# Sachin-A/TraceWeaver

Measured on NVIDIA H100. Metric: spans/sec reconstructed (in+out spans of all solved services), higher is better.
Workload: dtype int64 timestamps, f64 log-likelihoods

## Files before the change

traceweaver_b200/csrc/tw_gmm.cu:

```cuda
#include "tw_kernels.cuh"

namespace tw {

constexpr double kRegCovar = 1e-6;
constexpr double kEmTol = 1e-3;
constexpr int kEmMaxIter = 100;
constexpr int kKmMaxIter = 300;
constexpr double kKmTol = 1e-4;
constexpr double kDblEps = 2.220446049250313e-16;
constexpr int KC = TW_GMM_MAX_COMP;
constexpr unsigned kFull = 0xffffffffu;

#ifdef TW_PROFILE_PHASES
__device__ unsigned long long g_gmm_phase[16];
#define TW_GPHASE_BEGIN long long _gp_t0 = clock64()
#define TW_GPHASE_RESET _gp_t0 = clock64()
#define TW_GPHASE(k)                                                               \
  do {                                                                             \
    if ((threadIdx.x & 31) == 0) {                                                 \
      long long _now = clock64();                                                  \
      atomicAdd(&g_gmm_phase[k], (unsigned long long)(_now - _gp_t0));             \
      _gp_t0 = _now;                                                               \
    }                                                                              \
  } while (0)
#define TW_GCOUNT(k, v)                                                            \
  do {                                                                             \
    if ((threadIdx.x & 31) == 0) atomicAdd(&g_gmm_phase[k], (unsigned long long)(v)); \
  } while (0)
#else
#define TW_GPHASE_BEGIN do { } while (0)
#define TW_GPHASE_RESET do { } while (0)
#define TW_GPHASE(k) do { } while (0)
#define TW_GCOUNT(k, v) do { } while (0)
#endif

__device__ unsigned long long g_gmm_em_evals;

__device__ __forceinline__ double wsum(double v) {
#pragma unroll
  for (int d = 16; d > 0; d >>= 1) v += __shfl_xor_sync(kFull, v, d);
  return v;
}

__device__ __forceinline__ int trials_for_k(int k) { return k < 3 ? 2 : 3; }
__device__ __forceinline__ int draws_for_k(int k) { return 1 + (k - 1) * trials_for_k(k); }

__device__ __forceinline__ double sq_dist(double c, double c2, double x, double x2) {
  double d = dadd(dadd(dmul(-2.0, dmul(c, x)), c2), x2);
  return d > 0.0 ? d : 0.0;
}

struct Fit {
  double mu[KC], pc[KC], logpc[KC], logw[KC];
};

struct Near { double d; int j; };
__device__ __forceinline__ Near near_min(Near a, Near b) { return b.d < a.d ? b : a; }
template <int K>
__device__ __forceinline__ int nearest(const double* cen, double x) {
  Near v[KC];
#pragma unroll
  for (int j = 0; j < KC; ++j) {
    v[j].j = j;
    v[j].d = j < K ? dadd(dmul(cen[j], cen[j]), dmul(-2.0, dmul(x, cen[j]))) : 0.0;
  }
  if (K == 1) return 0;
  if (K == 2) return near_min(v[0], v[1]).j;
  if (K == 3) return near_min(near_min(v[0], v[1]), v[2]).j;
  if (K == 4) return near_min(near_min(v[0], v[1]), near_min(v[2], v[3])).j;
  return near_min(near_min(near_min(v[0], v[1]), near_min(v[2], v[3])), v[4]).j;
}

template <class F>
__device__ __forceinline__ void sweep2(const double* __restrict__ x, int n, F&& f) {
  int i = threadIdx.x & 31;
  double a = i < n ? x[i] : 0.0;
  double b = i + 32 < n ? x[i + 32] : 0.0;
  for (int s = 0; i < n; i += 64, s += 2) {
    const double x0 = a, x1 = b;
    const bool v1 = i + 32 < n;
    a = i + 64 < n ? x[i + 64] : 0.0;
    b = i + 96 < n ? x[i + 96] : 0.0;
    f(x0, x1, v1, s);
  }
}

template <int K>
__device__ __forceinline__ void seed_centres(const double* __restrict__ x, int n, double mean,
                                             const double* __restrict__ draws, double* cen) {
  const int lane = threadIdx.x & 31;
  const int k = K;
  TW_GPHASE_BEGIN;
#pragma unroll
  for (int j = 0; j < KC; ++j) cen[j] = 0.0;
  {
    double u = draws[0];
    double un = u * (double)n;
    int id = (int)un;
    if (fabs(un - rint(un)) < 1e-6) {
      double p = 1.0 / (double)n, last = 0.0, c = 0.0;
      for (int i = 0; i < n; ++i) last += p;
      id = n - 1;
      for (int i = 0; i < n; ++i) { c += p; if (c / last > u) { id = i; break; } }
    }
    if (id > n - 1) id = n - 1;
    cen[0] = x[id] - mean;
  }
  const int trials = trials_for_k(k);
  double pot = 0.0;
  {
    double part = 0.0, c2 = cen[0] * cen[0];
    for (int i = lane; i < n; i += 32) { double xi = x[i] - mean; part += sq_dist(cen[0], c2, xi, xi * xi); }
    pot = wsum(part);
  }
  for (int ci = 1; ci < k; ++ci) {
    double rv[3];
    int cand[3];
    for (int t = 0; t < 3; ++t) { rv[t] = t < trials ? draws[1 + (ci - 1) * trials + t] * pot : 0.0; cand[t] = n - 1; }
    bool found[3] = {false, false, false};
    double carry = 0.0;
    for (int base = 0; base < n; base += 32) {
      int i = base + lane;
      double cl = 0.0;
      if (i < n) {
        double xi = x[i] - mean, x2 = xi * xi;
        cl = sq_dist(cen[0], cen[0] * cen[0], xi, x2);
        for (int j = 1; j < ci; ++j) { double d = sq_dist(cen[j], cen[j] * cen[j], xi, x2); cl = d < cl ? d : cl; }
      }
      double incl = cl;
#pragma unroll
      for (int d = 1; d < 32; d <<= 1) {
        double o = __shfl_up_sync(kFull, incl, d);
        if (lane >= d) incl += o;
      }
      incl += carry;
      for (int t = 0; t < trials; ++t) {
        if (found[t]) continue;
        unsigned m = __ballot_sync(kFull, i < n && incl >= rv[t]);
        if (m) { cand[t] = base + __ffs(m) - 1; found[t] = true; }
      }
      carry = __shfl_sync(kFull, incl, 31);
      if (found[0] && (trials < 2 || found[1]) && (trials < 3 || found[2])) break;
    }
    double cc[3], part[3] = {0.0, 0.0, 0.0};
    for (int t = 0; t < 3; ++t) cc[t] = x[cand[t]] - mean;
    for (int i = lane; i < n; i += 32) {
      double xi = x[i] - mean, x2 = xi * xi;
      double cl = sq_dist(cen[0], cen[0] * cen[0], xi, x2);
      for (int j = 1; j < ci; ++j) { double d = sq_dist(cen[j], cen[j] * cen[j], xi, x2); cl = d < cl ? d : cl; }
      for (int t = 0; t < trials; ++t) {
        double d = sq_dist(cc[t], cc[t] * cc[t], xi, x2);
        part[t] += d < cl ? d : cl;
      }
    }
    int best = 0;
    double bp = wsum(part[0]);
    for (int t = 1; t < trials; ++t) {
      double pt = wsum(part[t]);
      if (pt < bp) { bp = pt; best = t; }
    }
    cen[ci] = cc[best];
    pot = bp;
  }
  TW_GPHASE(0);
}

template <int K>
__device__ __forceinline__ void lloyd_centres(const double* __restrict__ x, int n, double mean, double tol,
                                              const double* cen_in, double* cen_out) {
  const int lane = threadIdx.x & 31;
  const int k = K;
  TW_GPHASE_BEGIN;
  double cen[KC];
#pragma unroll
  for (int j = 0; j < KC; ++j) cen[j] = cen_in[j];
  double prev[KC];
#pragma unroll
  for (int j = 0; j < KC; ++j) prev[j] = cen[j];
  bool have_prev = false, strict = false;
  const bool packed = n <= 1024;
  unsigned long long lab_lo = 0ull, lab_hi = 0ull;
  for (int it = 0; it < kKmMaxIter; ++it) {
    double sx[KC];
    int cnt_i[KC];
#pragma unroll
    for (int j = 0; j < KC; ++j) { sx[j] = 0.0; cnt_i[j] = 0; }
    bool changed = !have_prev;
    if (packed) {
      sweep2(x, n, [&](double x0, double x1, bool v1, int s) {
#pragma unroll
        for (int h = 0; h < 2; ++h) {
          const double xi = (h ? x1 : x0) - mean;
          const bool valid = h ? v1 : true;
          const int lab = nearest<K>(cen, xi);
          const int sl = s + h;
          const unsigned sh = (unsigned)(sl & 15) * 4u;
          const bool hi = sl >= 16;
          const unsigned long long w = hi ? lab_hi : lab_lo;
          changed |= valid && (int)((w >> sh) & 15ull) != lab;
          const unsigned long long nw = valid ? (w & ~(15ull << sh)) | ((unsigned long long)lab << sh) : w;
          lab_lo = hi ? lab_lo : nw;
          lab_hi = hi ? nw : lab_hi;
#pragma unroll
          for (int j = 0; j < K; ++j) {
            const bool m = valid && j == lab;
            sx[j] += m ? xi : 0.0;
            cnt_i[j] += m ? 1 : 0;
          }
        }
      });
    } else {
      for (int i = lane; i < n; i += 32) {
        const double xi = x[i] - mean;
        const int lab = nearest<K>(cen, xi);
        if (have_prev && nearest<K>(prev, xi) != lab) changed = true;
#pragma unroll
        for (int j = 0; j < K; ++j) {
          const bool m = j == lab;
          sx[j] += m ? xi : 0.0;
          cnt_i[j] += m ? 1 : 0;
        }
      }
    }
    if (!have_prev) changed = true;
    double cnt[KC];
#pragma unroll
    for (int j = 0; j < KC; ++j) cnt[j] = (double)__reduce_add_sync(kFull, cnt_i[j]);
    changed = __any_sync(kFull, changed);
#pragma unroll
    for (int j = 0; j < KC; ++j) sx[j] = wsum(sx[j]);
    for (int j = 0; j < k; ++j) {
      if (cnt[j] != 0.0) continue;
      double fd = -1.0;
      int fi = 0x7fffffff;
      for (int i = lane; i < n; i += 32) {
        double xi = x[i] - mean;
        const int nl = nearest<K>(cen, xi);
        double cn = cen[0];
#pragma unroll
        for (int q = 1; q < KC; ++q) cn = q == nl ? cen[q] : cn;
        double d = xi - cn;
        d *= d;
        if (d > fd) { fd = d; fi = i; }
      }
#pragma unroll
      for (int d = 16; d > 0; d >>= 1) {
        double od = __shfl_xor_sync(kFull, fd, d);
        int oi = __shfl_xor_sync(kFull, fi, d);
        if (od > fd || (od == fd && oi < fi)) { fd = od; fi = oi; }
      }
      double xf = x[fi] - mean;
      int ol = nearest<K>(cen, xf);
#pragma unroll
      for (int q = 0; q < KC; ++q) {
        if (q == ol) { sx[q] -= xf; cnt[q] -= 1.0; }
        if (q == j) { sx[q] = xf; cnt[q] = 1.0; }
      }
    }
    double shift_tot = 0.0;
#pragma unroll
    for (int j = 0; j < KC; ++j) {
      prev[j] = cen[j];
      if (j < k) {
        double nc = cnt[j] > 0.0 ? sx[j] * (1.0 / cnt[j]) : sx[j];
        double d = fabs(nc - cen[j]);
        shift_tot += d * d;
        cen[j] = nc;
      }
    }
    have_prev = true;
    TW_GCOUNT(5, 1);
    if (!changed) { strict = true; break; }
    if (shift_tot <= tol) break;
  }
#pragma unroll
  for (int j = 0; j < KC; ++j) cen_out[j] = strict ? prev[j] : cen[j];
  TW_GPHASE(1);
}

template <bool FULL>
__device__ __forceinline__ bool params_from_stats(Fit& f, int k, int n, const double* nk, const double* mup,
                                                  const double* S2, double shift, bool init) {
  double tot = 0.0;
  bool ok = true;
#pragma unroll
  for (int c = 0; c < KC; ++c)
    if (c < k) tot += nk[c];
#pragma unroll
  for (int c = 0; c < KC; ++c) {
    if (c < k) {
      double cov = FULL ? S2[c] / nk[c] + kRegCovar : S2[c] / nk[c] - mup[c] * mup[c] + kRegCovar;
      if (!(cov > 0.0)) ok = false;
      f.mu[c] = mup[c] + shift;
      f.pc[c] = 1.0 / sqrt(cov);
      f.logpc[c] = log(f.pc[c]);
      f.logw[c] = log(init ? nk[c] / (double)n : nk[c] / tot);
    }
  }
  return ok;
}

template <int K, bool FULL>
__device__ __forceinline__ double estep(const Fit& f, const double* __restrict__ tab, double x, double* a,
                                        double* amax_out) {
  double amax = -INFINITY;
#pragma unroll
  for (int c = 0; c < K; ++c) {
#ifdef TW_GMM_FUSED
    const double y = (x - f.mu[c]) * f.pc[c];
    a[c] = fma(-0.5 * y, y, (f.logpc[c] - 0.5 * TW_LOG_2PI) + f.logw[c]);
#else
    double lp;
    if (FULL) {
      double y = dsub(dmul(x, f.pc[c]), dmul(f.mu[c], f.pc[c]));
      lp = dmul(y, y);
    } else {
      double prec = dmul(f.pc[c], f.pc[c]);
      lp = dadd(dsub(dmul(dmul(f.mu[c], f.mu[c]), prec), dmul(2.0, dmul(x, dmul(f.mu[c], prec)))),
                dmul(dmul(x, x), prec));
    }
    a[c] = dadd(dadd(dmul(-0.5, dadd(TW_LOG_2PI, lp)), f.logpc[c]), f.logw[c]);
#endif
    amax = a[c] > amax ? a[c] : amax;
  }
  double t = 0.0;
#pragma unroll
  for (int c = 0; c < K; ++c) {
    const double d = a[c] - amax;
    const double e = exp_neg(tab, d);
    a[c] = d >= -40.0 ? e : 0.0;
    t += a[c];
  }
  *amax_out = amax;
  return t;
}

struct LogSum {
  double acc = 0.0, prod = 1.0;
  int cnt = 0;
  __device__ __forceinline__ void add(double t, double amax) {
    acc += amax;
    prod *= t;
    if (++cnt == 128) { acc += log(prod); prod = 1.0; cnt = 0; }
  }
  __device__ __forceinline__ double total() const { return acc + log(prod); }
};

template <int K, bool FULL>
__device__ __forceinline__ bool em_fit(const double* __restrict__ x, int n, double mean, const double* cen,
                                       const double* __restrict__ tab, Fit& f, bool want_score, double* score) {
  const int lane = threadIdx.x & 31;
  const int k = K;
  if (n < 2 || n < k) return false;
  const double shift = FULL ? mean : 0.0;
  double S0[KC], S1[KC], S2[KC], nk[KC], mup[KC];
  TW_GPHASE_BEGIN;
  {
    TW_GCOUNT(7, 1);
#pragma unroll
    for (int c = 0; c < KC; ++c) { S0[c] = 0.0; S1[c] = 0.0; S2[c] = 0.0; }
    sweep2(x, n, [&](double x0, double x1, bool v1, int) {
#pragma unroll
      for (int h = 0; h < 2; ++h) {
        const double xi = h ? x1 : x0;
        const int lab = (h ? v1 : true) ? nearest<K>(cen, xi - mean) : -1;
        const double xs = xi - shift, xs2 = xs * xs;
#pragma unroll
        for (int c = 0; c < K; ++c) {
          const bool m = c == lab;
          S0[c] += m ? 1.0 : 0.0;
          S1[c] += m ? xs : 0.0;
          S2[c] += m ? xs2 : 0.0;
        }
      }
    });
#pragma unroll
    for (int c = 0; c < KC; ++c) {
      nk[c] = wsum(S0[c]) + 10.0 * kDblEps;
      mup[c] = wsum(S1[c]) / nk[c];
      S2[c] = wsum(S2[c]);
    }
    if (FULL) {
#pragma unroll
      for (int c = 0; c < KC; ++c) S2[c] = 0.0;
      sweep2(x, n, [&](double x0, double x1, bool v1, int) {
#pragma unroll
        for (int h = 0; h < 2; ++h) {
          const double xi = h ? x1 : x0;
          const int lab = (h ? v1 : true) ? nearest<K>(cen, xi - mean) : -1;
          const double xs = xi - shift;
#pragma unroll
          for (int c = 0; c < K; ++c) {
            const double d = xs - mup[c];
            S2[c] += c == lab ? d * d : 0.0;
          }
        }
      });
#pragma unroll
      for (int c = 0; c < KC; ++c) S2[c] = wsum(S2[c]);
    }
  }
  if (!params_from_stats<FULL>(f, k, n, nk, mup, S2, shift, true)) return false;
  TW_GPHASE(2);
  double lower = -INFINITY;
  int em_sweeps = 0;
  for (int it = 1; it <= kEmMaxIter; ++it) {
    const double prev = lower;
    LogSum ls;
#pragma unroll
    for (int c = 0; c < KC; ++c) { S0[c] = 0.0; S1[c] = 0.0; S2[c] = 0.0; }
    for (int i = lane; i < n; i += 32) {
      double xi = x[i], a[KC], amax;
      const double t = estep<K, FULL>(f, tab, xi, a, &amax);
      ls.add(t, amax);
      const double inv = 1.0 / t;
#pragma unroll
      for (int c = 0; c < K; ++c) {
        const double r = a[c] * inv;
        S0[c] += r;
        if (FULL) {
          const double dx = xi - f.mu[c];
          const double rd = r * dx;
          S1[c] += rd;
          S2[c] += rd * dx;
        } else {
          S1[c] += r * xi;
          S2[c] += r * (xi * xi);
        }
      }
    }
    lower = wsum(ls.total()) / (double)n;
#pragma unroll
    for (int c = 0; c < KC; ++c) {
      if (c < K) {
        nk[c] = wsum(S0[c]) + 10.0 * kDblEps;
        const double s1 = wsum(S1[c]);
        S2[c] = wsum(S2[c]);
        if (FULL) {
          const double delta = s1 / nk[c];
          S2[c] -= delta * s1;
          if (S2[c] < 0.0) S2[c] = 0.0;
          mup[c] = (f.mu[c] + delta) - shift;
        } else {
          mup[c] = s1 / nk[c];
        }
      }
    }
    if (!params_from_stats<FULL>(f, k, n, nk, mup, S2, shift, false)) {
      if (lane == 0) atomicAdd(&g_gmm_em_evals, (unsigned long long)it * (unsigned long long)n * K);
      return false;
    }
    TW_GCOUNT(6, 1);
    em_sweeps = it;
    if (fabs(lower - prev) < kEmTol) break;
  }
  if (lane == 0) atomicAdd(&g_gmm_em_evals, (unsigned long long)(em_sweeps + (want_score ? 1 : 0)) * (unsigned long long)n * K);
  TW_GPHASE(3);
  if (want_score) {
    LogSum ls;
    for (int i = lane; i < n; i += 32) {
      double a[KC], amax;
      const double t = estep<K, FULL>(f, tab, x[i], a, &amax);
      ls.add(t, amax);
    }
    *score = wsum(ls.total()) / (double)n;
  }
  TW_GPHASE(4);
  return true;
}

__global__ void __launch_bounds__(128)
k_gmm_prep(int n_terms, const int64_t* __restrict__ term_sample_off, const double* __restrict__ delays,
           const int32_t* __restrict__ counts, int32_t* __restrict__ max_n, double* __restrict__ mean_var) {
  const int t = (int)((blockIdx.x * (unsigned)blockDim.x + threadIdx.x) >> 5);
  const int lane = threadIdx.x & 31;
  if (t >= n_terms) return;
  const double* x = delays + term_sample_off[t];
  const int n = counts[t];
  double set[KC];
  int ns = 0;
  double part = 0.0;
  for (int i = lane; i < n; i += 32) {
    double v = x[i];
    part += v;
    bool seen = false;
#pragma unroll
    for (int q = 0; q < KC; ++q)
      if (q < ns && set[q] == v) seen = true;
    if (!seen && ns < KC) {
#pragma unroll
      for (int q = 0; q < KC; ++q)
        if (q == ns) set[q] = v;
      ++ns;
    }
  }
  double mset[KC];
  int mn = 0;
  for (int src = 0; src < 32 && mn < KC; ++src) {
    int sn = __shfl_sync(kFull, ns, src);
    for (int q = 0; q < KC; ++q) {
      double v = __shfl_sync(kFull, set[q < KC ? q : 0], src);
      if (q >= sn || mn >= KC) continue;
      bool seen = false;
#pragma unroll
      for (int r = 0; r < KC; ++r)
        if (r < mn && mset[r] == v) seen = true;
      if (!seen) {
#pragma unroll
        for (int r = 0; r < KC; ++r)
          if (r == mn) mset[r] = v;
        ++mn;
      }
    }
  }
  double mean = n > 0 ? wsum(part) / (double)n : 0.0;
  double p2 = 0.0;
  for (int i = lane; i < n; i += 32) { double d = x[i] - mean; p2 += d * d; }
  double var = n > 0 ? wsum(p2) / (double)n : 0.0;
  if (lane == 0) {
    max_n[t] = n > 0 ? mn : 0;
    mean_var[2 * t] = mean;
    mean_var[2 * t + 1] = var;
  }
}

__global__ void k_gmm_skip(int n_problems, const int32_t* __restrict__ prob_ep_off,
                           const int32_t* __restrict__ ep_term_off, const int32_t* __restrict__ term_order,
                           const int32_t* __restrict__ max_n, const uint32_t* __restrict__ prob_base_skip,
                           uint32_t* __restrict__ rng_skip) {
  int p = blockIdx.x * blockDim.x + threadIdx.x;
  if (p >= n_problems) return;
  int t0 = ep_term_off[prob_ep_off[p]], t1 = ep_term_off[prob_ep_off[p + 1]];
  uint32_t pos = prob_base_skip ? prob_base_skip[p] : 0u;
  for (int q = t0; q < t1; ++q) {
    int t = term_order ? term_order[q] : q;
    rng_skip[t] = pos;
    int mn = max_n[t];
    for (int k = 1; k <= mn; ++k) pos += (uint32_t)draws_for_k(k);
  }
}

__global__ void k_gmm_draws(int n_problems, const int32_t* __restrict__ prob_ep_off,
                            const int32_t* __restrict__ ep_term_off, const int32_t* __restrict__ max_n,
                            uint32_t* __restrict__ prob_draws) {
  int p = blockIdx.x * blockDim.x + threadIdx.x;
  if (p >= n_problems) return;
  uint32_t pos = 0;
  for (int t = ep_term_off[prob_ep_off[p]]; t < ep_term_off[prob_ep_off[p + 1]]; ++t)
    for (int k = 1; k <= max_n[t]; ++k) pos += (uint32_t)draws_for_k(k);
  prob_draws[p] = pos;
}

#ifndef TW_GMM_MINB
#define TW_GMM_MINB 1
#endif

struct FitSel {
  const int32_t* list;
  const uint32_t* hist;
  const int32_t* max_n;
  const uint32_t* rng_skip;
  const double* stream;
  int stream_len;
  int n_terms;
};

template <int K>
__device__ __forceinline__ bool select_fit(const FitSel& sel, const int32_t* __restrict__ counts, int* t_out,
                                           const double** draws_out, int* err_flag) {
  const unsigned w = (blockIdx.x * (unsigned)blockDim.x + threadIdx.x) >> 5;
  int t;
  const double* draws;
  if (sel.list) {
    if (w >= sel.hist[K]) return false;
    uint32_t off = 0;
#pragma unroll
    for (int q = 1; q < K; ++q) off += sel.hist[q];
    t = sel.list[off + w];
    draws = sel.stream;
  } else {
    if (w >= (unsigned)sel.n_terms) return false;
    t = (int)w;
    if (K > sel.max_n[t]) return false;
    uint32_t pos = sel.rng_skip[t];
#pragma unroll
    for (int q = 1; q < K; ++q) pos += (uint32_t)draws_for_k(q);
    if ((int)pos + draws_for_k(K) > sel.stream_len) {
      if (err_flag && (threadIdx.x & 31) == 0) atomicMin(err_flag, (int)TW_ERR_RANGE_LIMIT);
      return false;
    }
    draws = sel.stream + pos;
  }
  const int n = counts[t];
  if (n < 2 || n < K) return false;
  *t_out = t;
  *draws_out = draws;
  return true;
}

template <int K>
__global__ void __launch_bounds__(128)
k_gmm_seed(FitSel sel, const int64_t* __restrict__ term_sample_off, const double* __restrict__ delays,
           const int32_t* __restrict__ counts, const double* __restrict__ mean_var, double* __restrict__ cen_out,
           int* __restrict__ err_flag) {
  int t;
  const double* draws;
  if (!select_fit<K>(sel, counts, &t, &draws, err_flag)) return;
  double cen[KC];
  seed_centres<K>(delays + term_sample_off[t], counts[t], mean_var[2 * t], draws, cen);
  if ((threadIdx.x & 31) == 0) {
#pragma unroll
    for (int j = 0; j < K; ++j) cen_out[(size_t)t * KC + j] = cen[j];
  }
}

template <int K>
__global__ void __launch_bounds__(128)
k_gmm_lloyd(FitSel sel, const int64_t* __restrict__ term_sample_off, const double* __restrict__ delays,
            const int32_t* __restrict__ counts, const double* __restrict__ mean_var, double* __restrict__ cen_io) {
  int t;
  const double* draws;
  if (!select_fit<K>(sel, counts, &t, &draws, nullptr)) return;
  double cen[KC], out[KC];
#pragma unroll
  for (int j = 0; j < KC; ++j) cen[j] = j < K ? cen_io[(size_t)t * KC + j] : 0.0;
  lloyd_centres<K>(delays + term_sample_off[t], counts[t], mean_var[2 * t], mean_var[2 * t + 1] * kKmTol, cen, out);
  if ((threadIdx.x & 31) == 0) {
#pragma unroll
    for (int j = 0; j < K; ++j) cen_io[(size_t)t * KC + j] = out[j];
  }
}

template <int K>
__global__ void __launch_bounds__(128, TW_GMM_MINB)
k_gmm_bic(FitSel sel, const int64_t* __restrict__ term_sample_off, const double* __restrict__ delays,
          const int32_t* __restrict__ counts, const double* __restrict__ mean_var,
          const double* __restrict__ cen_in, double* __restrict__ bic_out) {
  __shared__ double tab[64];
  load_exp_table(tab);
  const int w = (int)((blockIdx.x * (unsigned)blockDim.x + threadIdx.x) >> 5);
  if (w >= sel.n_terms) return;
  double bic = INFINITY;
  int t;
  const double* draws;
  if (select_fit<K>(sel, counts, &t, &draws, nullptr)) {
    const int n = counts[t];
    double cen[KC];
#pragma unroll
    for (int j = 0; j < KC; ++j) cen[j] = j < K ? cen_in[(size_t)t * KC + j] : 0.0;
    Fit f;
    double sc = 0.0;
    if (em_fit<K, false>(delays + term_sample_off[t], n, mean_var[2 * t], cen, tab, f, true, &sc))
      bic = -2.0 * sc * (double)n + (double)(3 * K - 1) * log((double)n);
  }
  if ((threadIdx.x & 31) == 0) bic_out[(size_t)w * KC + (K - 1)] = bic;
}

__global__ void k_gmm_select(int n_terms, const int32_t* __restrict__ max_n, const double* __restrict__ bic,
                             int32_t* __restrict__ best_k_out, uint32_t* __restrict__ hist,
                             double* __restrict__ mix_out, int32_t* __restrict__ n_selected_out) {
  const int t = blockIdx.x * blockDim.x + threadIdx.x;
  if (t >= n_terms) return;
  int best_k = 0;
  double best = INFINITY;
  for (int k = 1; k <= max_n[t]; ++k) {
    double b = bic[(size_t)t * KC + (k - 1)];
    if (b < best) { best = b; best_k = k; }
  }
  best_k_out[t] = best_k;
  if (best_k > 0) atomicAdd(&hist[best_k], 1u);
  else {
    double* rec = mix_out + (size_t)t * TW_MIX_REC;
    for (int q = 0; q < TW_MIX_REC; ++q) rec[q] = 0.0;
    rec[2] = 0.001;
    rec[3] = log(0.001);
    if (n_selected_out) n_selected_out[t] = 0;
  }
}

__global__ void k_gmm_group(int n_terms, const int32_t* __restrict__ best_k, const uint32_t* __restrict__ hist,
                            uint32_t* __restrict__ cursor, int32_t* __restrict__ list) {
  const int t = blockIdx.x * blockDim.x + threadIdx.x;
  if (t >= n_terms) return;
  const int k = best_k[t];
  if (k <= 0) return;
  uint32_t off = 0;
  for (int q = 1; q < k; ++q) off += hist[q];
  list[off + atomicAdd(&cursor[k], 1u)] = t;
}

template <int K>
__global__ void __launch_bounds__(128, TW_GMM_MINB)
k_gmm_final(FitSel sel, const int64_t* __restrict__ term_sample_off, const double* __restrict__ delays,
            const int32_t* __restrict__ counts, const double* __restrict__ mean_var,
            const double* __restrict__ cen_in, double* __restrict__ mix_out, int32_t* __restrict__ n_selected_out) {
  __shared__ double tab[64];
  load_exp_table(tab);
  const unsigned w = (blockIdx.x * (unsigned)blockDim.x + threadIdx.x) >> 5;
  if (w >= sel.hist[K]) return;
  uint32_t off = 0;
#pragma unroll
  for (int q = 1; q < K; ++q) off += sel.hist[q];
  const int t = sel.list[off + w];
  const int lane = threadIdx.x & 31;
  const int n = counts[t];
  double cen[KC];
#pragma unroll
  for (int j = 0; j < KC; ++j) cen[j] = j < K ? cen_in[(size_t)t * KC + j] : 0.0;
  Fit f;
  const bool ok = em_fit<K, true>(delays + term_sample_off[t], n, mean_var[2 * t], cen, tab, f, false, nullptr);
  if (lane == 0) {
    double* rec = mix_out + (size_t)t * TW_MIX_REC;
    for (int q = 0; q < TW_MIX_REC; ++q) rec[q] = 0.0;
    if (ok) {
      rec[0] = (double)K;
#pragma unroll
      for (int c = 0; c < K; ++c) {
        rec[1 + c] = f.pc[c];
        rec[6 + c] = f.mu[c] * f.pc[c];
        rec[11 + c] = f.logpc[c];
        rec[16 + c] = f.logw[c];
      }
    } else {
      rec[2] = 0.001;
      rec[3] = log(0.001);
    }
    if (n_selected_out) n_selected_out[t] = ok ? K : 0;
  }
}

__global__ void __launch_bounds__(256)
k_fp64_peak(int iters, double* __restrict__ sink) {
  double a0 = threadIdx.x * 1e-9, a1 = a0 + 1e-3, a2 = a0 + 2e-3, a3 = a0 + 3e-3, a4 = a0 + 4e-3, a5 = a0 + 5e-3,
         a6 = a0 + 6e-3, a7 = a0 + 7e-3;
  const double m = 0.9999999, c = 1e-7;
  for (int i = 0; i < iters; ++i) {
    a0 = fma(a0, m, c); a1 = fma(a1, m, c); a2 = fma(a2, m, c); a3 = fma(a3, m, c);
    a4 = fma(a4, m, c); a5 = fma(a5, m, c); a6 = fma(a6, m, c); a7 = fma(a7, m, c);
  }
  const double r = ((a0 + a1) + (a2 + a3)) + ((a4 + a5) + (a6 + a7));
  if (r == 123.456) sink[0] = r;
}

cudaError_t launch_fp64_peak(int blocks, int iters, double* sink, cudaStream_t s, int64_t& launches) {
  k_fp64_peak<<<blocks, 256, 0, s>>>(iters, sink);
  return after_launch(launches);
}

cudaError_t gmm_work_read(unsigned long long* out, bool reset) {
  cudaError_t e = cudaMemcpyFromSymbol(out, g_gmm_em_evals, sizeof(unsigned long long));
  if (e != cudaSuccess) return e;
  if (reset) {
    const unsigned long long z = 0;
    e = cudaMemcpyToSymbol(g_gmm_em_evals, &z, sizeof z);
  }
  return e;
}

#ifdef TW_PROFILE_PHASES
extern "C" int tw_debug_gmm_phases(unsigned long long* out16, int reset) {
  cudaError_t e = cudaMemcpyFromSymbol(out16, g_gmm_phase, sizeof(unsigned long long) * 16);
  if (e != cudaSuccess) return -2;
  if (reset) {
    unsigned long long z[16] = {0};
    cudaMemcpyToSymbol(g_gmm_phase, z, sizeof z);
  }
  return 0;
}
#endif

cudaError_t launch_gmm_prep(int n_terms, const int64_t* term_sample_off, const double* delays,
                            const int32_t* counts, int32_t* max_n, double* mean_var, cudaStream_t s,
                            int64_t& launches) {
  k_gmm_prep<<<(n_terms + 3) / 4, 128, 0, s>>>(n_terms, term_sample_off, delays, counts, max_n, mean_var);
  return after_launch(launches);
}

cudaError_t launch_gmm_skip(int n_problems, const int32_t* prob_ep_off, const int32_t* ep_term_off,
                            const int32_t* term_order, const int32_t* max_n, const uint32_t* prob_base_skip,
                            uint32_t* rng_skip, cudaStream_t s, int64_t& launches) {
  k_gmm_skip<<<(n_problems + 127) / 128, 128, 0, s>>>(n_problems, prob_ep_off, ep_term_off, term_order, max_n,
                                                       prob_base_skip, rng_skip);
  return after_launch(launches);
}

cudaError_t launch_gmm_draws(int n_problems, const int32_t* prob_ep_off, const int32_t* ep_term_off,
                             const int32_t* max_n, uint32_t* prob_draws, cudaStream_t s, int64_t& launches) {
  k_gmm_draws<<<(n_problems + 127) / 128, 128, 0, s>>>(n_problems, prob_ep_off, ep_term_off, max_n, prob_draws);
  return after_launch(launches);
}

template <int K>
static cudaError_t launch_fit_phases(const FitSel& sel, int n_warps, const int64_t* term_sample_off,
                                     const double* delays, const int32_t* counts, const double* mean_var,
                                     double* cen, int* err_flag, cudaStream_t s, int64_t& launches) {
  const int blocks = (n_warps + 3) / 4;
  k_gmm_seed<K><<<blocks, 128, 0, s>>>(sel, term_sample_off, delays, counts, mean_var, cen, err_flag);
  cudaError_t e = after_launch(launches);
  if (e != cudaSuccess) return e;
  k_gmm_lloyd<K><<<blocks, 128, 0, s>>>(sel, term_sample_off, delays, counts, mean_var, cen);
  return after_launch(launches);
}

static cudaError_t fork_streams(GmmFork* fk, cudaStream_t s) {
  cudaError_t e = cudaEventRecord(fk->fork, s);
  for (int q = 0; q < TW_GMM_MAX_COMP && e == cudaSuccess; ++q) e = cudaStreamWaitEvent(fk->side[q], fk->fork, 0);
  return e;
}
static cudaError_t join_streams(GmmFork* fk, cudaStream_t s) {
  cudaError_t e = cudaSuccess;
  for (int q = 0; q < TW_GMM_MAX_COMP && e == cudaSuccess; ++q) {
    e = cudaEventRecord(fk->join[q], fk->side[q]);
    if (e == cudaSuccess) e = cudaStreamWaitEvent(s, fk->join[q], 0);
  }
  return e;
}

cudaError_t launch_gmm_fit(int n_terms, const int64_t* term_sample_off, const double* delays,
                           const int32_t* counts, const int32_t* max_n, const double* mean_var,
                           const uint32_t* rng_skip, const double* stream, int stream_len,
                           const double* stream100, double* bic, double* cen, double* mix_out,
                           int32_t* n_selected_out, int* err_flag, GmmFork* fk, cudaStream_t s,
                           int64_t& launches) {
  cudaError_t e;
  const int blocks = (n_terms + 3) / 4;
  const size_t slab = (size_t)n_terms * KC;
  const FitSel sel{nullptr, nullptr, max_n, rng_skip, stream, stream_len, n_terms};
  e = fork_streams(fk, s);
  if (e != cudaSuccess) return e;
#define TW_BIC(K)                                                                                          \
  {                                                                                                        \
    cudaStream_t q = fk->side[K - 1];                                                                      \
    double* c = cen + (K - 1) * slab;                                                                      \
    e = launch_fit_phases<K>(sel, n_terms, term_sample_off, delays, counts, mean_var, c, err_flag, q,      \
                             launches);                                                                    \
    if (e != cudaSuccess) return e;                                                                        \
    k_gmm_bic<K><<<blocks, 128, 0, q>>>(sel, term_sample_off, delays, counts, mean_var, c, bic);           \
    e = after_launch(launches);                                                                            \
    if (e != cudaSuccess) return e;                                                                        \
  }
  TW_BIC(5) TW_BIC(4) TW_BIC(3) TW_BIC(2) TW_BIC(1)
#undef TW_BIC
  e = join_streams(fk, s);
  if (e != cudaSuccess) return e;
  uint32_t* hist = const_cast<uint32_t*>(rng_skip);
  uint32_t* cursor = hist + 8;
  int32_t* best_k = const_cast<int32_t*>(max_n);
  int32_t* list = reinterpret_cast<int32_t*>(bic);
  e = cudaMemsetAsync(hist, 0, 16 * sizeof(uint32_t), s);
  if (e != cudaSuccess) return e;
  k_gmm_select<<<(n_terms + 127) / 128, 128, 0, s>>>(n_terms, max_n, bic, best_k, hist, mix_out, n_selected_out);
  e = after_launch(launches);
  if (e != cudaSuccess) return e;
  k_gmm_group<<<(n_terms + 127) / 128, 128, 0, s>>>(n_terms, best_k, hist, cursor, list);
  e = after_launch(launches);
  if (e != cudaSuccess) return e;
  const FitSel fin{list, hist, nullptr, nullptr, stream100, 16, n_terms};
  e = fork_streams(fk, s);
  if (e != cudaSuccess) return e;
#define TW_FINAL(K)                                                                                        \
  {                                                                                                        \
    cudaStream_t q = fk->side[K - 1];                                                                      \
    double* c = cen + (K - 1) * slab;                                                                      \
    e = launch_fit_phases<K>(fin, n_terms, term_sample_off, delays, counts, mean_var, c, nullptr, q,       \
                             launches);                                                                    \
    if (e != cudaSuccess) return e;                                                                        \
    k_gmm_final<K><<<blocks, 128, 0, q>>>(fin, term_sample_off, delays, counts, mean_var, c, mix_out,      \
                                          n_selected_out);                                                 \
    e = after_launch(launches);                                                                            \
    if (e != cudaSuccess) return e;                                                                        \
  }
  TW_FINAL(5) TW_FINAL(4) TW_FINAL(3) TW_FINAL(2) TW_FINAL(1)
#undef TW_FINAL
  return join_streams(fk, s);
}

}
```

Measured before the change: 490.8 million.

## Cache k-means++ nearest-centre distances in shared memory and launch one warp per block

k-means++ seeding now keeps each point's distance to its nearest chosen centre in a per-warp shared-memory array for samples up to 1024 points. Each new centre then updates that array once, instead of recomputing distances to every earlier centre in both the prefix-scan pass and the trial pass. All GMM kernels move from 128-thread blocks carrying four warps to 32-thread blocks carrying one warp, so the shared cache is private to each warp and finished warps release their slots sooner. The EM accumulation is pulled into a helper that uses explicit fma and intrinsic adds, which can change rounding slightly. Single-warp blocks raise the block count, and the 8 KB shared array per block may cap residency per SM.

```diff
diff --git a/traceweaver_b200/csrc/tw_gmm.cu b/traceweaver_b200/csrc/tw_gmm.cu
--- a/traceweaver_b200/csrc/tw_gmm.cu
+++ b/traceweaver_b200/csrc/tw_gmm.cu
@@ -85,11 +85,15 @@
   }
 }
 
+constexpr int kSeedCache = 1024;
+
 template <int K>
 __device__ __forceinline__ void seed_centres(const double* __restrict__ x, int n, double mean,
-                                             const double* __restrict__ draws, double* cen) {
+                                             const double* __restrict__ draws, double* cen,
+                                             double* __restrict__ closest) {
   const int lane = threadIdx.x & 31;
   const int k = K;
+  const bool cached = n <= kSeedCache;
   TW_GPHASE_BEGIN;
 #pragma unroll
   for (int j = 0; j < KC; ++j) cen[j] = 0.0;
@@ -110,9 +114,20 @@
   double pot = 0.0;
   {
     double part = 0.0, c2 = cen[0] * cen[0];
-    for (int i = lane; i < n; i += 32) { double xi = x[i] - mean; part += sq_dist(cen[0], c2, xi, xi * xi); }
+    for (int i = lane; i < n; i += 32) {
+      double xi = x[i] - mean;
+      const double d = sq_dist(cen[0], c2, xi, xi * xi);
+      if (cached) closest[i] = d;
+      part += d;
+    }
     pot = wsum(part);
   }
+  auto closest_to = [&](int i, int ci, double xi, double x2) {
+    if (cached) return closest[i];
+    double cl = sq_dist(cen[0], cen[0] * cen[0], xi, x2);
+    for (int j = 1; j < ci; ++j) { double d = sq_dist(cen[j], cen[j] * cen[j], xi, x2); cl = d < cl ? d : cl; }
+    return cl;
+  };
   for (int ci = 1; ci < k; ++ci) {
     double rv[3];
     int cand[3];
@@ -123,9 +138,8 @@
       int i = base + lane;
       double cl = 0.0;
       if (i < n) {
-        double xi = x[i] - mean, x2 = xi * xi;
-        cl = sq_dist(cen[0], cen[0] * cen[0], xi, x2);
-        for (int j = 1; j < ci; ++j) { double d = sq_dist(cen[j], cen[j] * cen[j], xi, x2); cl = d < cl ? d : cl; }
+        double xi = cached ? 0.0 : x[i] - mean;
+        cl = closest_to(i, ci, xi, xi * xi);
       }
       double incl = cl;
 #pragma unroll
@@ -146,8 +160,7 @@
     for (int t = 0; t < 3; ++t) cc[t] = x[cand[t]] - mean;
     for (int i = lane; i < n; i += 32) {
       double xi = x[i] - mean, x2 = xi * xi;
-      double cl = sq_dist(cen[0], cen[0] * cen[0], xi, x2);
-      for (int j = 1; j < ci; ++j) { double d = sq_dist(cen[j], cen[j] * cen[j], xi, x2); cl = d < cl ? d : cl; }
+      const double cl = closest_to(i, ci, xi, x2);
       for (int t = 0; t < trials; ++t) {
         double d = sq_dist(cc[t], cc[t] * cc[t], xi, x2);
         part[t] += d < cl ? d : cl;
@@ -161,6 +174,14 @@
     }
     cen[ci] = cc[best];
     pot = bp;
+    if (cached && ci + 1 < k) {
+      const double c2 = cen[ci] * cen[ci];
+      for (int i = lane; i < n; i += 32) {
+        double xi = x[i] - mean;
+        const double d = sq_dist(cen[ci], c2, xi, xi * xi);
+        closest[i] = d < closest[i] ? d : closest[i];
+      }
+    }
   }
   TW_GPHASE(0);
 }
@@ -335,6 +356,27 @@
   return t;
 }
 
+template <int K, bool FULL>
+__device__ __forceinline__ void mstep_add(const Fit& f, double xi, const double* a, double t, double* S0,
+                                          double* S1, double* S2) {
+  const double inv = 1.0 / t;
+  const double xi2 = dmul(xi, xi);
+#pragma unroll
+  for (int c = 0; c < K; ++c) {
+    const double r = dmul(a[c], inv);
+    S0[c] = dadd(S0[c], r);
+    if (FULL) {
+      const double dx = dsub(xi, f.mu[c]);
+      const double rd = dmul(r, dx);
+      S1[c] = dadd(S1[c], rd);
+      S2[c] = __fma_rn(rd, dx, S2[c]);
+    } else {
+      S1[c] = __fma_rn(r, xi, S1[c]);
+      S2[c] = __fma_rn(r, xi2, S2[c]);
+    }
+  }
+}
+
 struct LogSum {
   double acc = 0.0, prod = 1.0;
   int cnt = 0;
@@ -410,24 +452,11 @@
 #pragma unroll
     for (int c = 0; c < KC; ++c) { S0[c] = 0.0; S1[c] = 0.0; S2[c] = 0.0; }
     for (int i = lane; i < n; i += 32) {
-      double xi = x[i], a[KC], amax;
-      const double t = estep<K, FULL>(f, tab, xi, a, &amax);
-      ls.add(t, amax);
-      const double inv = 1.0 / t;
-#pragma unroll
-      for (int c = 0; c < K; ++c) {
-        const double r = a[c] * inv;
-        S0[c] += r;
-        if (FULL) {
-          const double dx = xi - f.mu[c];
-          const double rd = r * dx;
-          S1[c] += rd;
-          S2[c] += rd * dx;
-        } else {
-          S1[c] += r * xi;
-          S2[c] += r * (xi * xi);
-        }
-      }
+      double a0[KC], m0;
+      const double xi = x[i];
+      const double t0 = estep<K, FULL>(f, tab, xi, a0, &m0);
+      ls.add(t0, m0);
+      mstep_add<K, FULL>(f, xi, a0, t0, S0, S1, S2);
     }
     lower = wsum(ls.total()) / (double)n;
 #pragma unroll
@@ -459,9 +488,9 @@
   if (want_score) {
     LogSum ls;
     for (int i = lane; i < n; i += 32) {
-      double a[KC], amax;
-      const double t = estep<K, FULL>(f, tab, x[i], a, &amax);
-      ls.add(t, amax);
+      double a0[KC], m0;
+      const double t0 = estep<K, FULL>(f, tab, x[i], a0, &m0);
+      ls.add(t0, m0);
     }
     *score = wsum(ls.total()) / (double)n;
   }
@@ -551,9 +580,6 @@
   prob_draws[p] = pos;
 }
 
-#ifndef TW_GMM_MINB
-#define TW_GMM_MINB 1
-#endif
 
 struct FitSel {
   const int32_t* list;
@@ -599,15 +625,16 @@
 }
 
 template <int K>
-__global__ void __launch_bounds__(128)
+__global__ void __launch_bounds__(32)
 k_gmm_seed(FitSel sel, const int64_t* __restrict__ term_sample_off, const double* __restrict__ delays,
            const int32_t* __restrict__ counts, const double* __restrict__ mean_var, double* __restrict__ cen_out,
            int* __restrict__ err_flag) {
+  __shared__ double closest[kSeedCache];
   int t;
   const double* draws;
   if (!select_fit<K>(sel, counts, &t, &draws, err_flag)) return;
   double cen[KC];
-  seed_centres<K>(delays + term_sample_off[t], counts[t], mean_var[2 * t], draws, cen);
+  seed_centres<K>(delays + term_sample_off[t], counts[t], mean_var[2 * t], draws, cen, closest);
   if ((threadIdx.x & 31) == 0) {
 #pragma unroll
     for (int j = 0; j < K; ++j) cen_out[(size_t)t * KC + j] = cen[j];
@@ -615,7 +642,7 @@
 }
 
 template <int K>
-__global__ void __launch_bounds__(128)
+__global__ void __launch_bounds__(32)
 k_gmm_lloyd(FitSel sel, const int64_t* __restrict__ term_sample_off, const double* __restrict__ delays,
             const int32_t* __restrict__ counts, const double* __restrict__ mean_var, double* __restrict__ cen_io) {
   int t;
@@ -632,7 +659,7 @@
 }
 
 template <int K>
-__global__ void __launch_bounds__(128, TW_GMM_MINB)
+__global__ void __launch_bounds__(32)
 k_gmm_bic(FitSel sel, const int64_t* __restrict__ term_sample_off, const double* __restrict__ delays,
           const int32_t* __restrict__ counts, const double* __restrict__ mean_var,
           const double* __restrict__ cen_in, double* __restrict__ bic_out) {
@@ -690,7 +717,7 @@
 }
 
 template <int K>
-__global__ void __launch_bounds__(128, TW_GMM_MINB)
+__global__ void __launch_bounds__(32)
 k_gmm_final(FitSel sel, const int64_t* __restrict__ term_sample_off, const double* __restrict__ delays,
             const int32_t* __restrict__ counts, const double* __restrict__ mean_var,
             const double* __restrict__ cen_in, double* __restrict__ mix_out, int32_t* __restrict__ n_selected_out) {
@@ -794,11 +821,10 @@
 static cudaError_t launch_fit_phases(const FitSel& sel, int n_warps, const int64_t* term_sample_off,
                                      const double* delays, const int32_t* counts, const double* mean_var,
                                      double* cen, int* err_flag, cudaStream_t s, int64_t& launches) {
-  const int blocks = (n_warps + 3) / 4;
-  k_gmm_seed<K><<<blocks, 128, 0, s>>>(sel, term_sample_off, delays, counts, mean_var, cen, err_flag);
+  k_gmm_seed<K><<<n_warps, 32, 0, s>>>(sel, term_sample_off, delays, counts, mean_var, cen, err_flag);
   cudaError_t e = after_launch(launches);
   if (e != cudaSuccess) return e;
-  k_gmm_lloyd<K><<<blocks, 128, 0, s>>>(sel, term_sample_off, delays, counts, mean_var, cen);
+  k_gmm_lloyd<K><<<n_warps, 32, 0, s>>>(sel, term_sample_off, delays, counts, mean_var, cen);
   return after_launch(launches);
 }
 
@@ -823,7 +849,6 @@
                            int32_t* n_selected_out, int* err_flag, GmmFork* fk, cudaStream_t s,
                            int64_t& launches) {
   cudaError_t e;
-  const int blocks = (n_terms + 3) / 4;
   const size_t slab = (size_t)n_terms * KC;
   const FitSel sel{nullptr, nullptr, max_n, rng_skip, stream, stream_len, n_terms};
   e = fork_streams(fk, s);
@@ -835,7 +860,7 @@
     e = launch_fit_phases<K>(sel, n_terms, term_sample_off, delays, counts, mean_var, c, err_flag, q,      \
                              launches);                                                                    \
     if (e != cudaSuccess) return e;                                                                        \
-    k_gmm_bic<K><<<blocks, 128, 0, q>>>(sel, term_sample_off, delays, counts, mean_var, c, bic);           \
+    k_gmm_bic<K><<<n_terms, 32, 0, q>>>(sel, term_sample_off, delays, counts, mean_var, c, bic);           \
     e = after_launch(launches);                                                                            \
     if (e != cudaSuccess) return e;                                                                        \
   }
@@ -865,7 +890,7 @@
     e = launch_fit_phases<K>(fin, n_terms, term_sample_off, delays, counts, mean_var, c, nullptr, q,       \
                              launches);                                                                    \
     if (e != cudaSuccess) return e;                                                                        \
-    k_gmm_final<K><<<blocks, 128, 0, q>>>(fin, term_sample_off, delays, counts, mean_var, c, mix_out,      \
+    k_gmm_final<K><<<n_terms, 32, 0, q>>>(fin, term_sample_off, delays, counts, mean_var, c, mix_out,      \
                                           n_selected_out);                                                 \
     e = after_launch(launches);                                                                            \
     if (e != cudaSuccess) return e;                                                                        \
```

After: 491.1 million (median of 6 runs). About the same (+0.1%).

## Spread per-component GMM parameter updates across warp lanes with shared Fit

Applied to the files above, without the earlier changes.

Instead of every lane redundantly computing covariance, sqrt, division and two logs for all K components after each EM iteration, each lane now handles one component and writes into a per-warp Fit held in shared memory. This cuts redundant transcendental work and register pressure, and launch bounds now ask for 4 blocks per SM for K>=4 in place of a fixed macro. In exchange the estep reads parameters from shared memory and adds warp syncs and an all-vote, and the explicitly rounded intrinsics are meant to keep the numerics unchanged.

```diff
diff --git a/traceweaver_b200/csrc/tw_gmm.cu b/traceweaver_b200/csrc/tw_gmm.cu
--- a/traceweaver_b200/csrc/tw_gmm.cu
+++ b/traceweaver_b200/csrc/tw_gmm.cu
@@ -278,26 +278,35 @@
   TW_GPHASE(1);
 }
 
-template <bool FULL>
-__device__ __forceinline__ bool params_from_stats(Fit& f, int k, int n, const double* nk, const double* mup,
-                                                  const double* S2, double shift, bool init) {
-  double tot = 0.0;
+template <int K>
+__device__ __forceinline__ double lane_component(const double* v) {
+  const int lane = threadIdx.x & 31;
+  double r = v[0];
+#pragma unroll
+  for (int c = 1; c < K; ++c) r = lane == c ? v[c] : r;
+  return r;
+}
+
+template <int K, bool FULL>
+__device__ __forceinline__ bool params_from_stats(Fit& f, int n, double nk, double mup, double S2, double tot,
+                                                  double shift, bool init) {
+  const int c = threadIdx.x & 31;
   bool ok = true;
-#pragma unroll
-  for (int c = 0; c < KC; ++c)
-    if (c < k) tot += nk[c];
-#pragma unroll
-  for (int c = 0; c < KC; ++c) {
-    if (c < k) {
-      double cov = FULL ? S2[c] / nk[c] + kRegCovar : S2[c] / nk[c] - mup[c] * mup[c] + kRegCovar;
-      if (!(cov > 0.0)) ok = false;
-      f.mu[c] = mup[c] + shift;
-      f.pc[c] = 1.0 / sqrt(cov);
-      f.logpc[c] = log(f.pc[c]);
-      f.logw[c] = log(init ? nk[c] / (double)n : nk[c] / tot);
-    }
-  }
-  return ok;
+  __syncwarp();
+  if (c < K) {
+    const double q = __ddiv_rn(S2, nk);
+    const double cov = FULL     ? __dadd_rn(q, kRegCovar)
+                       : c == 0 ? __dadd_rn(fma(-mup, mup, q), kRegCovar)
+                                : __dadd_rn(__dsub_rn(q, __dmul_rn(mup, mup)), kRegCovar);
+    ok = cov > 0.0;
+    const double pc = __ddiv_rn(1.0, sqrt(cov));
+    f.mu[c] = __dadd_rn(mup, shift);
+    f.pc[c] = pc;
+    f.logpc[c] = log(pc);
+    f.logw[c] = log(__ddiv_rn(nk, init ? (double)n : tot));
+  }
+  __syncwarp();
+  return __all_sync(kFull, ok);
 }
 
 template <int K, bool FULL>
@@ -354,6 +363,7 @@
   if (n < 2 || n < k) return false;
   const double shift = FULL ? mean : 0.0;
   double S0[KC], S1[KC], S2[KC], nk[KC], mup[KC];
+  double my_nk, my_mup, my_s2;
   TW_GPHASE_BEGIN;
   {
     TW_GCOUNT(7, 1);
@@ -375,12 +385,16 @@
       }
     });
 #pragma unroll
-    for (int c = 0; c < KC; ++c) {
+    for (int c = 0; c < K; ++c) {
       nk[c] = wsum(S0[c]) + 10.0 * kDblEps;
-      mup[c] = wsum(S1[c]) / nk[c];
+      S1[c] = wsum(S1[c]);
       S2[c] = wsum(S2[c]);
     }
+    my_nk = lane_component<K>(nk);
+    my_mup = __ddiv_rn(lane_component<K>(S1), my_nk);
     if (FULL) {
+#pragma unroll
+      for (int c = 0; c < K; ++c) mup[c] = __shfl_sync(kFull, my_mup, c);
 #pragma unroll
       for (int c = 0; c < KC; ++c) S2[c] = 0.0;
       sweep2(x, n, [&](double x0, double x1, bool v1, int) {
@@ -397,10 +411,11 @@
         }
       });
 #pragma unroll
-      for (int c = 0; c < KC; ++c) S2[c] = wsum(S2[c]);
-    }
-  }
-  if (!params_from_stats<FULL>(f, k, n, nk, mup, S2, shift, true)) return false;
+      for (int c = 0; c < K; ++c) S2[c] = wsum(S2[c]);
+    }
+    my_s2 = lane_component<K>(S2);
+  }
+  if (!params_from_stats<K, FULL>(f, n, my_nk, my_mup, my_s2, 0.0, shift, true)) return false;
   TW_GPHASE(2);
   double lower = -INFINITY;
   int em_sweeps = 0;
@@ -430,23 +445,26 @@
       }
     }
     lower = wsum(ls.total()) / (double)n;
-#pragma unroll
-    for (int c = 0; c < KC; ++c) {
-      if (c < K) {
-        nk[c] = wsum(S0[c]) + 10.0 * kDblEps;
-        const double s1 = wsum(S1[c]);
-        S2[c] = wsum(S2[c]);
-        if (FULL) {
-          const double delta = s1 / nk[c];
-          S2[c] -= delta * s1;
-          if (S2[c] < 0.0) S2[c] = 0.0;
-          mup[c] = (f.mu[c] + delta) - shift;
-        } else {
-          mup[c] = s1 / nk[c];
-        }
-      }
-    }
-    if (!params_from_stats<FULL>(f, k, n, nk, mup, S2, shift, false)) {
+    double tot = 0.0;
+#pragma unroll
+    for (int c = 0; c < K; ++c) {
+      nk[c] = wsum(S0[c]) + 10.0 * kDblEps;
+      tot += nk[c];
+      S1[c] = wsum(S1[c]);
+      S2[c] = wsum(S2[c]);
+    }
+    my_nk = lane_component<K>(nk);
+    const double s1 = lane_component<K>(S1);
+    my_s2 = lane_component<K>(S2);
+    if (FULL) {
+      const double delta = __ddiv_rn(s1, my_nk);
+      my_s2 = fma(-delta, s1, my_s2);
+      if (my_s2 < 0.0) my_s2 = 0.0;
+      my_mup = __dsub_rn(__dadd_rn(f.mu[lane < K ? lane : 0], delta), shift);
+    } else {
+      my_mup = __ddiv_rn(s1, my_nk);
+    }
+    if (!params_from_stats<K, FULL>(f, n, my_nk, my_mup, my_s2, tot, shift, false)) {
       if (lane == 0) atomicAdd(&g_gmm_em_evals, (unsigned long long)it * (unsigned long long)n * K);
       return false;
     }
@@ -551,9 +569,7 @@
   prob_draws[p] = pos;
 }
 
-#ifndef TW_GMM_MINB
-#define TW_GMM_MINB 1
-#endif
+constexpr int em_min_blocks(int K) { return K >= 4 ? 4 : 1; }
 
 struct FitSel {
   const int32_t* list;
@@ -632,11 +648,12 @@
 }
 
 template <int K>
-__global__ void __launch_bounds__(128, TW_GMM_MINB)
+__global__ void __launch_bounds__(128, em_min_blocks(K))
 k_gmm_bic(FitSel sel, const int64_t* __restrict__ term_sample_off, const double* __restrict__ delays,
           const int32_t* __restrict__ counts, const double* __restrict__ mean_var,
           const double* __restrict__ cen_in, double* __restrict__ bic_out) {
   __shared__ double tab[64];
+  __shared__ Fit fits[128 / 32];
   load_exp_table(tab);
   const int w = (int)((blockIdx.x * (unsigned)blockDim.x + threadIdx.x) >> 5);
   if (w >= sel.n_terms) return;
@@ -648,7 +665,7 @@
     double cen[KC];
 #pragma unroll
     for (int j = 0; j < KC; ++j) cen[j] = j < K ? cen_in[(size_t)t * KC + j] : 0.0;
-    Fit f;
+    Fit& f = fits[threadIdx.x >> 5];
     double sc = 0.0;
     if (em_fit<K, false>(delays + term_sample_off[t], n, mean_var[2 * t], cen, tab, f, true, &sc))
       bic = -2.0 * sc * (double)n + (double)(3 * K - 1) * log((double)n);
@@ -690,11 +707,12 @@
 }
 
 template <int K>
-__global__ void __launch_bounds__(128, TW_GMM_MINB)
+__global__ void __launch_bounds__(128, em_min_blocks(K))
 k_gmm_final(FitSel sel, const int64_t* __restrict__ term_sample_off, const double* __restrict__ delays,
             const int32_t* __restrict__ counts, const double* __restrict__ mean_var,
             const double* __restrict__ cen_in, double* __restrict__ mix_out, int32_t* __restrict__ n_selected_out) {
   __shared__ double tab[64];
+  __shared__ Fit fits[128 / 32];
   load_exp_table(tab);
   const unsigned w = (blockIdx.x * (unsigned)blockDim.x + threadIdx.x) >> 5;
   if (w >= sel.hist[K]) return;
@@ -707,7 +725,7 @@
   double cen[KC];
 #pragma unroll
   for (int j = 0; j < KC; ++j) cen[j] = j < K ? cen_in[(size_t)t * KC + j] : 0.0;
-  Fit f;
+  Fit& f = fits[threadIdx.x >> 5];
   const bool ok = em_fit<K, true>(delays + term_sample_off[t], n, mean_var[2 * t], cen, tab, f, false, nullptr);
   if (lane == 0) {
     double* rec = mix_out + (size_t)t * TW_MIX_REC;
```

New measurement: 471.3 million before, 488.7 million after (median of 6 runs). 1.04x the previous value.
